# agordon/fastx_toolkit

Hardware: AMD Instinct MI355X
Metric: Mreads/s (150 bp) quality-trim+filter (higher is better)
Workload: dtype u8

## Files before the change

fastx_toolkit_amd/build.py:

```python
import os
import shutil
import subprocess
import sys

PKG = os.path.dirname(os.path.abspath(__file__))
ROOT = os.path.dirname(PKG)
CSRC = os.path.join(PKG, "csrc")
HOST = os.path.join(PKG, "host")
LIBFXG = os.path.join(PKG, "libfxg.so")

HIPCC_FLAGS = ["--offload-arch=gfx950", "-O3", "-std=c++17", "-ffp-contract=off", "-fPIC", "-shared"]


def _newer(target, deps):
    if not os.path.exists(target):
        return True
    t = os.path.getmtime(target)
    return any(os.path.getmtime(d) > t for d in deps if os.path.exists(d))


def hipcc():
    exe = shutil.which("hipcc") or "/opt/rocm/bin/hipcc"
    if not os.path.exists(exe):
        raise RuntimeError("hipcc not found: the gfx950 engine cannot be built")
    return exe


def check_exec_zero(so):
    tool = os.path.join(ROOT, "scripts", "check_exec_zero.py")
    p = subprocess.run([sys.executable, tool, so], stdout=subprocess.PIPE, stderr=subprocess.STDOUT, text=True)
    if p.returncode not in (0, 1):
        raise RuntimeError("%s NOT CHECKED: scripts/check_exec_zero.py could not read the library's ISA (exit code %d); that is a broken check, "
                           "not a finding, and a library that was not checked is not accepted.\n%s" % (so, p.returncode, p.stdout[-3000:]))
    if p.returncode != 0:
        raise RuntimeError("%s REJECTED: vector/memory code runs with EXEC = 0 at the exit of a lane-divergent loop (compiler bug, DESIGN.md section 3).\n"
                           "Change the register budget of the named instance (fxg_clip_waves / __launch_bounds__) or its source and rebuild.\n%s" % (so, p.stdout[-3000:]))


CLIP_UNITS = 7


def compile_engine(out, extra_flags=(), check=True):
    tmp = out + ".new"
    objdir = os.path.join(ROOT, "build", "engine_" + os.path.basename(out).replace(".", "_"))
    os.makedirs(objdir, exist_ok=True)
    cflags = [f for f in HIPCC_FLAGS if f != "-shared"] + list(extra_flags) + ["-c"]
    units = [("fxg_engine.hip", ["-DFXG_SPLIT"], os.path.join(objdir, "engine.o"))]
    units += [("fxg_engine_clip.hip", ["-DFXG_CLIP_TU=%d" % k], os.path.join(objdir, "clip%d.o" % k)) for k in range(1, CLIP_UNITS + 1)]
    procs = [(src, subprocess.Popen([hipcc()] + cflags + defs + [os.path.join(CSRC, src), "-o", obj])) for src, defs, obj in units]
    failed = [src for src, p in procs if p.wait() != 0]
    if failed:
        raise RuntimeError("hipcc failed on %s" % ", ".join(failed))
    subprocess.check_call([hipcc(), "--offload-arch=gfx950", "-fPIC", "-shared"] + [obj for _, _, obj in units] + ["-o", tmp])
    if check:
        try:
            check_exec_zero(tmp)
        except Exception:
            os.replace(tmp, out + ".rejected")
            raise
    os.replace(tmp, out)
    return out


def build_engine(force=False):
    deps = [os.path.join(CSRC, f) for f in os.listdir(CSRC)] + [os.path.join(ROOT, "include", "fxg.h")]
    if force or _newer(LIBFXG, deps):
        compile_engine(LIBFXG)
    return LIBFXG


def build_host(force=False):
    mk = os.path.join(HOST, "Makefile")
    if os.path.exists(mk):
        subprocess.check_call(["make", "-s", "-C", HOST] + (["-B"] if force else []))


def build_all(force=False):
    build_engine(force)
    build_host(force)
    return LIBFXG
```

fastx_toolkit_amd/csrc/fxg_device.h:

```cpp
#pragma once
#include <hip/hip_runtime.h>
#include <stdint.h>
#include <cstdio>
#include <cstring>

#include "../../include/fxg.h"

typedef unsigned int       u32;
typedef unsigned long long u64;
typedef unsigned int u32x4 __attribute__((ext_vector_type(4)));

#define FXG_HD __host__ __device__ __forceinline__
#define FXG_PLAN_FAIL(...) do { snprintf(err, cap, __VA_ARGS__); return FXG_E_INVALID; } while (0)
static inline int fxg_text_check_len(unsigned long long text_len, char *err, size_t cap) { if (text_len > 0xFFFFFFF0ull) FXG_PLAN_FAIL("text block too large (%llu bytes)", text_len); return FXG_OK; }
static inline bool fxg_text_lpr_ok(int lpr) { return lpr == 4 || lpr == 2; }

#if defined(FXG_ABLATION) || defined(FXG_DBG_BITS)
#define FXG_DBG(a, bit) ((a).debug & (bit))
#else
#define FXG_DBG(a, bit) 0u
#endif

#define FXG_BLOCK 256
#define FXG_WAVES (FXG_BLOCK / 64)
// ... 410 lines not shown
    return lane < 2u ? fxg_granule_load(a.pfx + 2 * (u64)tile + lane) : ((u64)a.tag << FXG_TAG_SHIFT);
}
__device__ __forceinline__ void fxg_wait_prefix(const FxgKArgs &a, u32 tile, u64 peek, u64 *bc)
{
    const u32 lane = fxg_lane();
    u64 v = peek;
    u32 spins = 0;
    const u64 t0 = __builtin_amdgcn_s_memrealtime();
    while (__ballot((u32)(v >> FXG_TAG_SHIFT) != a.tag) != 0ull) {
        __builtin_amdgcn_s_sleep(1);
        if (lane < 2u) v = fxg_granule_load(a.pfx + 2 * (u64)tile + lane);
        if ((++spins & 255u) == 0u && fxg_spin_expired(a, t0)) break;
    }
    const bool ok = __ballot((u32)(v >> FXG_TAG_SHIFT) != a.tag) == 0ull;
    if (lane < 2u) bc[lane] = ok ? FXG_TAG_VALUE(v) : ~0ull;
}

#ifndef FXG_POLL_SLEEP
#define FXG_POLL_SLEEP 1
#endif
__device__ __forceinline__ void fxg_wait_prefix_wave(const FxgKArgs &a, u32 tile, u64 *bc)
{
    const u32 lane = fxg_lane();
    u64 v = fxg_peek_prefix(a, tile);
    u32 spins = 0;
    const u64 t0 = __builtin_amdgcn_s_memrealtime();
    while (__ballot((u32)(v >> FXG_TAG_SHIFT) != a.tag) != 0ull) {
        __builtin_amdgcn_s_sleep(FXG_POLL_SLEEP);
        if (lane < 2u) v = fxg_granule_load(a.pfx + 2 * (u64)tile + lane);
        if ((++spins & 255u) == 0u && fxg_spin_expired(a, t0)) break;
    }
    const bool ok = __ballot((u32)(v >> FXG_TAG_SHIFT) != a.tag) == 0ull;
    v = ok ? FXG_TAG_VALUE(v) : ~0ull;
    bc[0] = ((u64)(u32)__builtin_amdgcn_readlane((int)(v >> 32), 0) << 32) | (u32)__builtin_amdgcn_readlane((int)(u32)v, 0);
    bc[1] = ((u64)(u32)__builtin_amdgcn_readlane((int)(v >> 32), 1) << 32) | (u32)__builtin_amdgcn_readlane((int)(u32)v, 1);
}

template <int TW = FXG_TWAVES>
__device__ __forceinline__ void fxg_block_scan2(u32 c, u32 b, u32 *scratch, u32 *ex_c, u32 *ex_b, u32 *tot_c, u32 *tot_b)
{
    const u32 lane = fxg_lane(), wave = threadIdx.x >> 6;
    const u32 ic = fxg_wave_scan_dpp(c), ib = fxg_wave_scan_dpp(b);
    if constexpr (TW == 1) {
        *ex_c = ic - c; *ex_b = ib - b;
        *tot_c = (u32)__builtin_amdgcn_readlane((int)ic, 63); *tot_b = (u32)__builtin_amdgcn_readlane((int)ib, 63);
        return;
    }
    if (lane == 63) { scratch[wave] = ic; scratch[TW + wave] = ib; }
    __syncthreads();
    u32 oc = 0, ob = 0, sc = 0, sb = 0;
#pragma unroll
    for (int w = 0; w < TW; ++w) {
// ... 181 lines not shown
```

fastx_toolkit_amd/csrc/fxg_engine.hip:

```cpp
#include "fxg_host.h"
#include "fxg_text.h"
#include "fxg_history.h"
#include "fxg_stats.h"
#include "fxg_fallback.h"
#include "fxg_barcode.h"
#include "fxg_reflow.h"

extern "C" int fxg_abi_version(void) { return FXG_ABI_VERSION; }

extern "C" int fxg_ctx_create(int device_id, fxg_ctx **out)
{
    if (!out) return FXG_E_INVALID;
    *out = nullptr;
    int ndev = 0;
    if (hipGetDeviceCount(&ndev) != hipSuccess || ndev <= 0 || device_id < 0 || device_id >= ndev) return FXG_E_HIP;
    fxg_ctx *c = (fxg_ctx *)calloc(1, sizeof(fxg_ctx));
    if (!c) return FXG_E_NOMEM;
    c->device = device_id;
    hipDeviceProp_t prop;
    if (hipSetDevice(device_id) != hipSuccess || hipGetDeviceProperties(&prop, device_id) != hipSuccess ||
        hipStreamCreateWithFlags(&c->own_stream, hipStreamNonBlocking) != hipSuccess) { fxg_ctx_destroy(c); return FXG_E_HIP; }
    c->cus = prop.multiProcessorCount;
    c->stream = c->own_stream;
    { const char *e = getenv("FXG_BLOCKS_PER_CU"); c->env_blocks_per_cu = (e && atoi(e) > 0 && atoi(e) <= 16) ? atoi(e) : 0; }
// ... 162 lines not shown
    }
    if (hist) {
        FXG_HIP(c, hipSetDevice(c->device));
        FXG_TRY(fxg_hist_prepass(c, in, estride, pl));
    }
    c->fb_req.valid = 0;
    if (pl.ka.compact) { c->fb_req.in = *in; c->fb_req.p = *p; c->fb_req.out = *out; c->fb_req.hist = hist; c->fb_req.estride = estride; c->fb_req.valid = 1; }
    return fxg_launch_plan(c, pl, (u64 *)out->counters);
}

static int fxg_launch_clip(fxg_ctx *c, FxgPlan &pl, u64 *ctr)
{
    int rc;
#define FXG_CLIP_TRY_UNIT(K) if ((rc = FXG_CLIP_UNIT_FN(K)(c, pl, ctr)) != FXG_CLIP_NOT_MINE) return rc;
    FXG_CLIP_FOR_UNITS(FXG_CLIP_TRY_UNIT)
#undef FXG_CLIP_TRY_UNIT
    return fxg_fail(c, FXG_E_INVALID, "no clip instance %d", pl.amax);
}

static int fxg_launch_plan(fxg_ctx *c, FxgPlan &pl, u64 *ctr)
{
    if (pl.rows_nw) {
        if (pl.rows_h == 2) {
            if (pl.rows_nw == 26) return fxg_launch_tiles(c, fxg_kernel_rows<26, 2>, "fxg_kernel_rows<26,2> qtrim+qfilter", pl.ka, pl.lds, ctr, 64u, true);
            return fxg_launch_tiles(c, fxg_kernel_rows<38, 2>, "fxg_kernel_rows<38,2> qtrim+qfilter", pl.ka, pl.lds, ctr, 64u, true);
        }
        switch (pl.rows_nw) {
        case 10: return fxg_launch_tiles(c, fxg_kernel_rows_multi<10, 4>, "fxg_kernel_rows_multi<10,4> qtrim+qfilter", pl.ka, pl.lds, ctr, 64u, true);
        case 14: return fxg_launch_tiles(c, fxg_kernel_rows_multi<14, 3>, "fxg_kernel_rows_multi<14,3> qtrim+qfilter", pl.ka, pl.lds, ctr, 64u, true);
        case 20: return fxg_launch_tiles(c, fxg_kernel_rows_multi<20, 2>, "fxg_kernel_rows_multi<20,2> qtrim+qfilter", pl.ka, pl.lds, ctr, 64u, true);
        case 26: return fxg_launch_tiles(c, fxg_kernel_rows<26>, "fxg_kernel_rows<26> qtrim+qfilter", pl.ka, pl.lds, ctr, 64u, true);
        default: return fxg_launch_tiles(c, fxg_kernel_rows<38>, "fxg_kernel_rows<38> qtrim+qfilter", pl.ka, pl.lds, ctr, 64u, true);
        }
    }
    if (pl.group_a) {
        if (pl.amax == 0) return fxg_launch_tiles(c, fxg_kernel_tiles<0, 0>, "fxg_kernel_tiles<0,0> qtrim+qfilter", pl.ka, pl.lds, ctr);
        return fxg_launch_clip(c, pl, ctr);
    }
    if (pl.mask) return fxg_launch_tiles(c, fxg_kernel_tiles<0, 3>, "fxg_kernel_tiles<0,3> mask", pl.ka, pl.lds, ctr);
    if (pl.artifacts) return fxg_launch_tiles(c, fxg_kernel_tiles<0, 4>, "fxg_kernel_tiles<0,4> base census", pl.ka, pl.lds, ctr);
    if (pl.rev && pl.ka.rev_dw) return fxg_launch_tiles(c, fxg_kernel_tiles<0, 5>, "fxg_kernel_tiles<0,5> revcomp[+ftrim], dword-aligned windows", pl.ka, pl.lds, ctr);
    if (pl.rev) return fxg_launch_tiles(c, fxg_kernel_tiles<0, 2>, "fxg_kernel_tiles<0,2> revcomp[+ftrim]", pl.ka, pl.lds, ctr);
    return fxg_launch_tiles(c, fxg_kernel_tiles<0, 1>, "fxg_kernel_tiles<0,1> ftrim", pl.ka, pl.lds, ctr);
}

extern "C" int fxg_run_quality_stats(fxg_ctx *c, const fxg_batch *in, uint64_t *d_hist, uint32_t hist_cols)
{
    if (!c) return FXG_E_INVALID;
    FXG_TRY(fxg_stats_check(in, d_hist, hist_cols, c->err, sizeof c->err));
    if (in->n == 0) return FXG_OK;
    FXG_HIP(c, hipSetDevice(c->device));
    u64 nwg = (in->n + 255) / 256;
    if (nwg > (u64)c->cus) nwg = (u64)c->cus;
    FxgStatsArgs a = fxg_stats_args(in, d_hist, hist_cols, (u32)nwg);
    const size_t need = (size_t)a.nwg * FXG_QS_PART_WORDS;
// ... 523 lines not shown
```

fastx_toolkit_amd/csrc/fxg_engine_clip.hip:

```cpp
#include "fxg_host.h"

#define FXG_CLIP_LAUNCH(K, NAME) return fxg_launch_tiles(c, K, NAME, pl.ka, pl.lds, ctr, pl.block, false, pl.ck_per_wg);
#define FXG_CLIP_CASE_PACKED(N) case -N: FXG_CLIP_LAUNCH((pl.ka.clip_global ? fxg_kernel_tiles<-N, 0, true> : fxg_kernel_tiles<-N, 0, false>), "fxg_kernel_tiles<-" #N ",0> clip(packed)[+qtrim+qfilter]")
#define FXG_CLIP_CASE_GENERAL(N) case N: FXG_CLIP_LAUNCH((fxg_kernel_tiles<N, 0>), "fxg_kernel_tiles<" #N ",0> clip[+qtrim+qfilter]")
#define FXG_CLIP_DEFINE_UNIT(K) \
    int FXG_CLIP_UNIT_FN(K)(fxg_ctx *c, FxgPlan &pl, u64 *ctr) { switch (pl.amax) { FXG_CLIP_UNIT(K)(FXG_CLIP_CASE_PACKED, FXG_CLIP_CASE_GENERAL) default: return FXG_CLIP_NOT_MINE; } }

#ifdef FXG_CLIP_TU
FXG_CLIP_DEFINE_UNIT(FXG_CLIP_TU)
#else
FXG_CLIP_FOR_UNITS(FXG_CLIP_DEFINE_UNIT)
#endif
```

fastx_toolkit_amd/csrc/fxg_host.h:

```cpp
#pragma once
#include <hip/hip_runtime.h>

#include <dlfcn.h>
#include <fcntl.h>
#include <cerrno>
#include <cstdarg>
#include <cstdio>
#include <cstdlib>
#include <cstring>
#include <unistd.h>

#include "fxg_plan.h"
#include "fxg_rows.h"

struct FxgTextState;

struct fxg_ctx {
    int device;
    int cus;
    hipStream_t own_stream;
    hipStream_t stream;
    hipEvent_t ev0, ev1;
#define FXG_KEV_RING 64
    hipEvent_t kev0[FXG_KEV_RING], kev1[FXG_KEV_RING];
// ... 89 lines not shown
template <typename K>
static int fxg_kernel_fit(fxg_ctx *c, K kernel, const char *kname, u32 lds, int *per_cu, u32 block = FXG_TBLOCK)
{
    for (int i = 0; i < 8; ++i)
        if (c->attr_kernel[i] == (void *)kernel && c->attr_lds[i] == lds) { *per_cu = c->attr_per_cu[i]; return FXG_OK; }
    int k = -1;
    for (int i = 0; i < 32; ++i) { if (c->lds_kernel[i] == (void *)kernel) { k = i; break; } if (!c->lds_kernel[i] && k < 0) k = i; }
    if (k < 0 || c->lds_kernel[k] != (void *)kernel || c->lds_max[k] < lds) {
        FXG_HIP(c, hipFuncSetAttribute((const void *)kernel, hipFuncAttributeMaxDynamicSharedMemorySize, (int)lds));
        if (k >= 0) { c->lds_kernel[k] = (void *)kernel; c->lds_max[k] = lds; }
    }
    FXG_HIP(c, hipOccupancyMaxActiveBlocksPerMultiprocessor(per_cu, kernel, (int)block, lds));
    if (*per_cu < 1) return fxg_fail(c, FXG_E_INVALID, "%s does not fit on a CU (lds=%u)", kname, lds);
    int slot = -1;
    for (int i = 0; i < 8; ++i) if (!c->attr_kernel[i]) { slot = i; break; }
    if (slot < 0) { slot = c->attr_next; c->attr_next = (c->attr_next + 1) % 8; }
    c->attr_kernel[slot] = (void *)kernel; c->attr_lds[slot] = lds; c->attr_per_cu[slot] = *per_cu;
    return FXG_OK;
}

#define FXG_STATUS_WORDS(cap) (3 * (size_t)(cap) + 2 * ((size_t)(cap) / 256 + 2))

template <typename K>
static int fxg_launch_tiles(fxg_ctx *c, K kernel, const char *kname, FxgKArgs &ka, u32 lds, u64 *counters, u32 block = FXG_TBLOCK, bool rows_kernel = false, u64 ck_per_wg = 0)
{
    FXG_HIP(c, hipSetDevice(c->device));
    int per_cu = 0;
    FXG_TRY(fxg_kernel_fit(c, kernel, kname, lds, &per_cu, block));
    const int most = block == 64u ? 16 : 8;
    int use = per_cu > most ? most : per_cu;
    if (c->env_blocks_per_cu > 0) use = c->env_blocks_per_cu;
    u64 workers = (u64)c->cus * (u64)use;
    if (c->env_workers > 0 && workers > (u64)c->env_workers) workers = (u64)c->env_workers;
    if (workers > ka.ntiles) workers = ka.ntiles;
    if (workers < 1) workers = 1;
    ka.nscan = !ka.compact ? 0u : (rows_kernel && workers >= 64u * FXG_ROWS_NSCAN ? (u32)FXG_ROWS_NSCAN : 1u);
    if (ka.compact && rows_kernel && c->env_nscan > 0) ka.nscan = (u32)c->env_nscan;
    const u64 grid = workers + ka.nscan;

    if (ka.compact) {
        bool fresh = false;
        const size_t cap = (size_t)ka.ntiles + (size_t)ka.ntiles / 4 + 1024;
        FXG_TRY(fxg_ws_grow(c, c->status, c->status_cap, ka.ntiles, cap, &fresh, FXG_STATUS_WORDS(cap) * sizeof(u64)));
        c->epoch = c->epoch >= 255u ? 1u : c->epoch + 1u;
        if (fresh || c->epoch == 1u) FXG_HIP(c, hipMemsetAsync(c->status, 0, FXG_STATUS_WORDS(c->status_cap) * sizeof(u64), c->stream));
        ka.agg = c->status;
        ka.pfx = c->status + c->status_cap;
        ka.bbase = c->status + 3 * c->status_cap;
        ka.tag = c->epoch;
    }
    ka.clip_ck = nullptr;
    if (ck_per_wg) {
// ... 32 lines not shown
```

fastx_toolkit_amd/csrc/fxg_plan.h:

```cpp
#pragma once
#include <cstdio>
#include <cstdlib>
#include <cstring>

#include "fxg_clip_instances.h"
#include "fxg_kernels.h"
#include "fxg_rows.h"

static_assert(fxg_clip_bucket(1) != 0 && fxg_clip_bucket(FXG_MAX_ADAPTER) != 0, "every adapter length the plan accepts needs a packed clip instance");

struct FxgPlan {
    FxgKArgs ka;
    bool group_a;
    bool clip, use_q, rev;
    bool mask, artifacts;
    int  amax;
    u32  lds;
    int  rows_nw;
    int  rows_h;
    int  rows_r;
    u32  block;
    u64  ck_per_wg;
};

static inline int fxg_clampi(long long v, int lo, int hi) { return v < lo ? lo : (v > hi ? hi : (int)v); }

static inline u32 fxg_pick_tile(u32 stride, bool clip, u32 block = FXG_TBLOCK)
{
    const u64 budget = clip ? 60ull * 1024 : 20ull * 1024;
    u32 T = block;
    const char *env = getenv("FXG_TILE");
    if (env && atoi(env) >= 1 && atoi(env) <= (int)block && (atoi(env) & (atoi(env) - 1)) == 0) return (u32)atoi(env);
    while (T > 1 && (u64)T * stride > budget) T >>= 1;
    return T;
}

static inline FxgLds fxg_plan_layout(const FxgPlan *pl)
{
    const FxgKArgs &ka = pl->ka;
    return pl->group_a ? fxg_lds_layout(ka.tile_reads, ka.stride, fxg_bitmap_count(ka, pl->use_q, pl->clip), (pl->clip && !ka.clip_global) ? ka.clip_stride : 0u, pl->clip ? ka.depth : 2u, pl->clip,
                                        (pl->clip && fxg_clip_uses_ptab(pl->amax)) ? fxg_ptab_bytes(ka.clip_ptab_rows, ka.clip_ptab_stride) : 0u)
         : pl->mask ? fxg_lds_layout(ka.tile_reads, ka.stride, 2u, 0u)
         : pl->artifacts ? fxg_lds_layout(ka.tile_reads, ka.stride, 4u, 0u) : fxg_lds_layout(ka.tile_reads, ka.stride, 0u, 0u);
// ... 66 lines not shown
        pl->amax = -b;
        if (two_pass_k) pl->ck_per_wg = (u64)FXG_CK_SLOTS * (u64)b * FXG_TBLOCK;
        ka.clip_ptab_cols = kform ? ((u32)b + 3u) & ~3u : 16u;
        ka.clip_ptab_stride = fxg_ptab_stride(ka.clip_ptab_cols);
        ka.clip_ptab_dia1 = kform ? FXG_K_DIA1 : FXG_PK_DIA1;
        if (kform && ka.clip_ptab_rows > FXG_PTAB_MAX_ROWS_K) {
            pl->amax = ka.alen <= 32 ? 32 : ka.alen <= 64 ? 64 : 100;
            pl->ck_per_wg = 0;
        }
    }
    pl->rows_nw = 0; pl->rows_h = 1; pl->rows_r = 1;
    {
        const int want = getenv("FXG_ROWS") ? atoi(getenv("FXG_ROWS")) : 1;
        const u32 top = want >= 2 ? 304u : 208u;
        if (ga && !pl->clip && ka.compact && in->stride >= 80u && in->stride <= top && want != 0) {
            pl->rows_h = in->stride <= 152u ? 1 : 2;
            pl->rows_nw = in->stride <= 104u * (u32)pl->rows_h ? 26 : 38;
        } else if (ga && !pl->clip && ka.compact && in->stride >= 28u && in->stride < 80u && want != 0) {
            if (in->stride <= 40u) { pl->rows_nw = 10; pl->rows_r = 4; }
            else if (in->stride <= 56u) { pl->rows_nw = 14; pl->rows_r = 3; }
            else { pl->rows_nw = 20; pl->rows_r = 2; }
        }
    }
    pl->block = pl->rows_nw ? 64u : (ga && pl->amax < 0 && pl->amax >= -16) ? (u32)FXG_CLIP_TBLOCK : (u32)FXG_TBLOCK;
    ka.clip_global = 0u;
    u32 T = pl->rows_nw ? 64u * (u32)pl->rows_r / (u32)pl->rows_h : fxg_pick_tile(pl->clip ? ka.clip_stride : in->stride, pl->clip, pl->block);
    if (pl->clip && pl->amax < 0 && (pl->amax >= -16 || pl->ck_per_wg != 0) && clip_stride == 0u && (ka.clip_stride & 3u) == 0u && ((uintptr_t)ka.clip_src & 3u) == 0u) {
        ka.tile_reads = T; ka.depth = 2u;
        const bool cramped = T < pl->block || (156u * 1024u) / fxg_plan_lds(pl) < 3u;
        const char *e = getenv("FXG_CLIP_GLOBAL");
        ka.clip_global = (e ? atoi(e) != 0 : cramped) ? 1u : 0u;
        if (ka.clip_global) T = pl->block;
    }
    const u64 ntiles = (in->n + T - 1) / T;
    if (ntiles > 0x7FFFFFFFull || in->n > 0xFFFFFFFFull) FXG_PLAN_FAIL("batch too large (%llu reads): split it", (unsigned long long)in->n);
    ka.tile_reads = T; ka.ntiles = (u32)ntiles;
    ka.rev_dw = 0u;
    if ((st & FXG_STAGE_REVCOMP) && !in->len && (T & 3u) == 0u) {
        u32 start = 0, cur = in->fixed_len;
        if (st & FXG_STAGE_FTRIM) {
            if (p->ft_last != 0 && (u32)p->ft_last < cur) cur = (u32)p->ft_last;
            if (p->ft_first != 1 && cur >= (u32)p->ft_first) { start = (u32)p->ft_first - 1u; cur -= start; }
        }
        if ((st & FXG_STAGE_FTRIM_END) && cur > p->ft_trim_end) cur -= p->ft_trim_end;
        const u32 A = (in->stride + cur) & 3u, C = (in->fixed_len - start) & 3u;
        ka.rev_dw = ((A == 0u && C != 0u) || (A == 2u && (C & 1u))) ? 1u : 0u;
// ... 36 lines not shown
```

fastx_toolkit_amd/csrc/fxg_rows.h:

```cpp
#pragma once
#include "fxg_kernels.h"

#define FXG_ROWS_T 64u
#ifndef FXG_ROWS_LB
#define FXG_ROWS_LB 3
#endif
#ifndef FXG_ROWS_SCAN_K
#define FXG_ROWS_SCAN_K 8
#endif
#ifndef FXG_ROWS_LD_AUX
#define FXG_ROWS_LD_AUX 2
#endif
#ifndef FXG_ROWS_NSCAN
#define FXG_ROWS_NSCAN 8
#endif
#ifndef FXG_ROWS_SPARSE_BASES
#define FXG_ROWS_SPARSE_BASES 1
#endif
#define FXG_ROWS_SPARSE_MULTI (FXG_ROWS_SPARSE_BASES >= 2)

__host__ __device__ inline u32 fxg_rows_lds(u32 stride, u32 lanes_per_read = 1u, u32 reads_per_lane = 1u) { return fxg_r16(FXG_ROWS_T * reads_per_lane / lanes_per_read * stride) + 176u; }

template <int NW>
FXG_HD void fxg_rows_bits(const u32 (&row)[NW], u32 K, u32 (&M)[(NW * 4 + 31) / 32])
{
#pragma unroll
    for (int p = 0; p < (NW + 1) / 2; ++p) {
        const u32 f0 = fxg_ge_flags(row[2 * p], K), f1 = 2 * p + 1 < NW ? fxg_ge_flags(row[2 * p + 1], K) : 0u;
#ifndef FXG_HOST_EMULATION
// ... 225 lines not shown
    const u32 first = sh ? 1u : 0u, end = (sh + totb) >> 4;
    const u32 s2 = (16u - sh) & 15u, qd = s2 >> 2, r = s2 & 3u;
    const int a8 = (int)(((base - sh) >> 4) & 7u);
    for (int ii = (int)lane - a8; ii < (int)end; ii += 64) {
        if (ii < (int)first) continue;
        const u32 i = (u32)ii;
        const u32x4 *src = reinterpret_cast<const u32x4 *>(obuf + ((i - first) << 4));
        const u32x4 v0 = src[0], v1 = src[1];
        u32 w0, w1, w2, w3, w4;
        if (qd == 0u)      { w0 = v0.x; w1 = v0.y; w2 = v0.z; w3 = v0.w; w4 = v1.x; }
        else if (qd == 1u) { w0 = v0.y; w1 = v0.z; w2 = v0.w; w3 = v1.x; w4 = v1.y; }
        else if (qd == 2u) { w0 = v0.z; w1 = v0.w; w2 = v1.x; w3 = v1.y; w4 = v1.z; }
        else               { w0 = v0.w; w1 = v1.x; w2 = v1.y; w3 = v1.z; w4 = v1.w; }
        const u32x4 o = {__builtin_amdgcn_alignbyte(w1, w0, r), __builtin_amdgcn_alignbyte(w2, w1, r), __builtin_amdgcn_alignbyte(w3, w2, r), __builtin_amdgcn_alignbyte(w4, w3, r)};
        fxg_st16_stream(g0 + ((u64)i << 4), o);
    }
    const bool whole = end > first;
    const u32 hb = whole ? (sh ? 16u - sh : 0u) : totb;
    const u32 ts = whole ? (end << 4) - sh : totb;
    if (lane < hb) out[base + lane] = obuf[lane];
    if (ts + lane < totb) out[base + ts + lane] = obuf[ts + lane];
}

#ifdef FXG_ABLATION
#define FXG_PHASE(i) do { const u64 now_ = __builtin_amdgcn_s_memrealtime(); ph[i] += now_ - pt; pt = now_; } while (0)
#else
#define FXG_PHASE(i) do { } while (0)
#endif

template <int NW, int H = 1>
__global__ __launch_bounds__(64, FXG_ROWS_LB) void fxg_kernel_rows(const FxgKArgs a)
{
    constexpr u32 TR = FXG_ROWS_T / (u32)H, HB = 4u * (u32)NW;
    extern __shared__ __attribute__((aligned(16))) unsigned char smem[];
    fxg_lds_u8 *lsm = (fxg_lds_u8 *)smem;
    u32 lane = threadIdx.x;
    const u32 stride = a.stride;
#if FXG_ROWS_SPARSE_BASES
    const u32 magic = fxg_rows_magic(stride);
#endif
    u32 role = 0;
    if (lane == 0) role = atomicAdd(a.role, 1u);
    role = (u32)__builtin_amdgcn_readfirstlane((int)role);
    if (role < a.nscan) { if (a.nscan == 1u) fxg_scanner_k<FXG_ROWS_SCAN_K>(a); else fxg_scanner_multi<FXG_ROWS_SCAN_K>(a, role); return; }
    const u32 G = a.ticket_groups, grp = blockIdx.x % G;
    u32 *my_ticket = a.ticket + grp * FXG_TICKET_STRIDE;
    u32 tk = 0;
    if (lane == 0) tk = atomicAdd(my_ticket, 1u);
    u32 cur = (u32)__builtin_amdgcn_readfirstlane((int)tk) * G + grp;
    u64 t_in = 0, t_kept = 0, t_bases = 0, t_qtrim = 0, t_qfilter = 0;
#ifdef FXG_ABLATION
    u64 ph[8] = {0, 0, 0, 0, 0, 0, 0, 0}, pt = __builtin_amdgcn_s_memrealtime();
#endif
    u32 qp[NW];
    u32 p_info = 0, p_exc = 0, p_totb = 0, pend = FXG_NO_TILE;
    for (;;) {
        asm volatile("" : "+v"(lane));
        const bool havec = cur < a.ntiles, havep = pend != FXG_NO_TILE;
        u32 q[NW];
        u32 c_info = 0, c_exc = 0, c_totb = 0;
        if (havec) {
            const u32 r0 = cur * TR;
            const u64 left = a.n - (u64)r0;
            const u32 nreads = left < (u64)TR ? (u32)left : TR;
            const u64 tb = (u64)r0 * stride;
            const u32 tbytes = nreads * stride;
            const u32 rd = lane / (u32)H, hf = lane % (u32)H;
            fxg_rows_fetch<NW>(a.qual, tb, tbytes, lsm, lane);
            fxg_rows_landed();
            FXG_PHASE(0);
            fxg_rows_read<NW>(smem, rd * stride + hf * HB, q);
            FXG_WAVE_SYNC();
            u32 keep = 0, olen = 0, word = 0;
            if constexpr (H == 1) {
                if (lane < nreads) word = fxg_rows_decide<NW>(a, q, r0 + lane, &keep, &olen);
            } else {
                constexpr int NM = (NW * 4 + 31) / 32;
                const bool live = rd < nreads;
                const u32 rl = live ? (a.len ? (u32)a.len[r0 + rd] : a.fixed_len) : 0u;
                u32 G[NM];
                const u32 kp = fxg_rows_piece_last<NW>(a, q, fxg_rows_piece_len(rl, HB, hf), G);
                const u32 ko = (u32)__builtin_amdgcn_mov_dpp((int)kp, 0xB1, 0xf, 0xf, true);
                const u32 k_lo = hf ? ko : kp, k_hi = hf ? kp : ko;
                const u32 k = k_hi ? HB + k_hi : k_lo;
                const u32 cl = (a.stages & FXG_STAGE_QTRIM) ? k : rl;
                const u32 lp = fxg_rows_piece_low<NW>(a, q, G, fxg_rows_piece_len(cl, HB, hf));
                const u32 lo_ = (u32)__builtin_amdgcn_mov_dpp((int)lp, 0xB1, 0xf, 0xf, true);
                u32 rlen = 0;
                word = fxg_rows_verdict(a, rl, k, lp + lo_, &keep, &rlen);
                if (!live) { keep = 0; word = 0; }
                if (live && hf == 0u) a.res[r0 + rd] = word;
                olen = keep ? fxg_rows_piece_len(rlen, HB, hf) : 0u;
                if (hf) word = 0;
            }
            {
                const u32 why = (H == 1 ? lane < nreads : rd < nreads) ? (word >> 17) & 0xFu : 0u;
                t_qtrim += (u64)__builtin_popcountll(__ballot(why == FXG_R_QTRIM));
                t_qfilter += (u64)__builtin_popcountll(__ballot(why == FXG_R_QFILTER));
            }
            const u32 mine = keep ? ((hf == 0u ? 1u << 16 : 0u) | olen) : 0u;
            const u32 inc = fxg_wave_scan_dpp(mine);
            const u32 tot = (u32)__builtin_amdgcn_readlane((int)inc, 63);
            const u32 totc = tot >> 16;
            c_totb = tot & 0xFFFFu;
            c_exc = (inc - mine) >> 16;
            c_info = ((keep && (H == 1 || hf == 0u || olen)) ? 1u << 31 : 0u) | (olen << 16) | ((inc - mine) & 0xFFFFu);
            if (lane == 0) fxg_publish_total(a, cur, totc, c_totb);
            t_in += nreads; t_kept += totc; t_bases += c_totb;
            FXG_PHASE(1);
        }
        u64 bc[2] = {0, 0};
        if (havep) {
            if (!FXG_DBG(a, 2u)) fxg_wait_prefix_wave(a, pend, bc); else { bc[0] = (u64)pend * TR; bc[1] = bc[0] * stride; }
            FXG_PHASE(2);
        }
        u32 nxt = 0;
        if (havec && lane == 0) nxt = atomicAdd(my_ticket, 1u);
        if (havep) {
            const u32 r0 = pend * TR;
            const u64 left = a.n - (u64)r0;
            const u32 nreads = left < (u64)TR ? (u32)left : TR;
            const u64 tb = (u64)r0 * stride;
            const u32 tbytes = nreads * stride;
            const u32 rd = lane / (u32)H, hf = lane % (u32)H;
            const bool placed = bc[0] != ~0ull;
            const u32 keep = placed ? p_info >> 31 : 0u, olen = (p_info >> 16) & 0x7FFFu, exb = p_info & 0xFFFFu;
            const bool fast = __ballot(keep && olen < 4u) == 0ull;
            if (keep && !FXG_DBG(a, 64u)) fxg_rows_pack<NW>(smem, exb, qp, olen, fast);
            FXG_WAVE_SYNC();
            FXG_PHASE(6);
            if (placed && !FXG_DBG(a, 1u)) fxg_rows_flush(a.out_qual, bc[1], p_totb, smem, lane);
// ... 17 lines not shown
#endif
                fxg_rows_fetch<NW, FXG_ROWS_SPARSE_BASES != 0>(a.bases, tb, tbytes, lsm, lane, need);
                fxg_rows_landed();
                FXG_PHASE(4);
                fxg_rows_read<NW>(smem, rd * stride + hf * HB, b);
                FXG_WAVE_SYNC();
                if (keep && !FXG_DBG(a, 64u)) fxg_rows_pack<NW>(smem, exb, b, olen, fast);
                FXG_WAVE_SYNC();
                FXG_PHASE(7);
                if (placed && !FXG_DBG(a, 1u)) fxg_rows_flush(a.out_bases, bc[1], p_totb, smem, lane);
                FXG_WAVE_SYNC();
            }
            FXG_PHASE(5);
        }
        if (!havec) break;
#pragma unroll
        for (int k = 0; k < NW; ++k) qp[k] = q[k];
        p_info = c_info; p_exc = c_exc; p_totb = c_totb; pend = cur;
        cur = (u32)__builtin_amdgcn_readfirstlane((int)nxt) * G + grp;
    }
#ifdef FXG_ABLATION
    if (lane == 0) for (int i = 0; i < 8; ++i) atomicAdd(reinterpret_cast<u64 *>(a.errflag + 10) + i, ph[i]);
#endif
    if (lane == 0) {
        if (t_in) atomicAdd(&a.tally[0], t_in);
        if (t_kept) atomicAdd(&a.tally[1], t_kept);
        if (t_bases) atomicAdd(&a.tally[2], t_bases);
        if (t_qtrim) atomicAdd(&a.tally[4 + FXG_R_QTRIM], t_qtrim);
        if (t_qfilter) atomicAdd(&a.tally[4 + FXG_R_QFILTER], t_qfilter);
    }
}
template <int NW, int R>
__global__ __launch_bounds__(64, FXG_ROWS_LB) void fxg_kernel_rows_multi(const FxgKArgs a)
{
    constexpr u32 TR = FXG_ROWS_T * (u32)R;
    extern __shared__ __attribute__((aligned(16))) unsigned char smem[];
    fxg_lds_u8 *lsm = (fxg_lds_u8 *)smem;
    u32 lane = threadIdx.x;
    const u32 stride = a.stride;
#if FXG_ROWS_SPARSE_MULTI
    const u32 magic = fxg_rows_magic(stride);
#endif
    u32 role = 0;
    if (lane == 0) role = atomicAdd(a.role, 1u);
    role = (u32)__builtin_amdgcn_readfirstlane((int)role);
    if (role < a.nscan) { if (a.nscan == 1u) fxg_scanner_k<FXG_ROWS_SCAN_K>(a); else fxg_scanner_multi<FXG_ROWS_SCAN_K>(a, role); return; }
    const u32 G = a.ticket_groups, grp = blockIdx.x % G;
    u32 *my_ticket = a.ticket + grp * FXG_TICKET_STRIDE;
    u32 tk = 0;
    if (lane == 0) tk = atomicAdd(my_ticket, 1u);
    u32 cur = (u32)__builtin_amdgcn_readfirstlane((int)tk) * G + grp;
    u64 t_in = 0, t_kept = 0, t_bases = 0, t_qtrim = 0, t_qfilter = 0;
    u32 qp[R][NW];
    u32 p_info[R], p_exc[R], p_totb = 0, pend = FXG_NO_TILE;
#pragma unroll
    for (int j = 0; j < R; ++j) { p_info[j] = 0u; p_exc[j] = 0u; }
    for (;;) {
        asm volatile("" : "+v"(lane));
        const bool havec = cur < a.ntiles, havep = pend != FXG_NO_TILE;
        u32 q[R][NW];
        u32 c_info[R], c_exc[R], c_totb = 0;
#pragma unroll
        for (int j = 0; j < R; ++j) { c_info[j] = 0u; c_exc[j] = 0u; }
        if (havec) {
            const u32 r0 = cur * TR;
            const u64 left = a.n - (u64)r0;
            const u32 nreads = left < (u64)TR ? (u32)left : TR;
            const u64 tb = (u64)r0 * stride;
            const u32 tbytes = nreads * stride;
            fxg_rows_fetch<NW * R>(a.qual, tb, tbytes, lsm, lane);
            fxg_rows_landed();
#pragma unroll
            for (int j = 0; j < R; ++j) fxg_rows_read<NW>(smem, ((u32)j * FXG_ROWS_T + lane) * stride, q[j]);
            FXG_WAVE_SYNC();
            u32 base = 0;
#pragma unroll
            for (int j = 0; j < R; ++j) {
                const u32 rd = (u32)j * FXG_ROWS_T + lane;
                u32 keep = 0, olen = 0, word = 0;
                if (rd < nreads) word = fxg_rows_decide<NW>(a, q[j], r0 + rd, &keep, &olen);
                const u32 why = rd < nreads ? (word >> 17) & 0xFu : 0u;
                t_qtrim += (u64)__builtin_popcountll(__ballot(why == FXG_R_QTRIM));
                t_qfilter += (u64)__builtin_popcountll(__ballot(why == FXG_R_QFILTER));
                const u32 mine = keep ? ((1u << 16) | olen) : 0u;
                const u32 inc = fxg_wave_scan_dpp(mine);
                const u32 ex = inc - mine + base;
                base += (u32)__builtin_amdgcn_readlane((int)inc, 63);
                c_exc[j] = ex >> 16;
                c_info[j] = (keep ? 1u << 31 : 0u) | (olen << 16) | (ex & 0xFFFFu);
            }
            const u32 totc = base >> 16;
            c_totb = base & 0xFFFFu;
            if (lane == 0) fxg_publish_total(a, cur, totc, c_totb);
            t_in += nreads; t_kept += totc; t_bases += c_totb;
        }
        u64 bc[2] = {0, 0};
        if (havep) fxg_wait_prefix_wave(a, pend, bc);
        u32 nxt = 0;
        if (havec && lane == 0) nxt = atomicAdd(my_ticket, 1u);
        if (havep) {
            const u32 r0 = pend * TR;
            const u64 left = a.n - (u64)r0;
            const u32 nreads = left < (u64)TR ? (u32)left : TR;
            const u64 tb = (u64)r0 * stride;
            const u32 tbytes = nreads * stride;
            const bool placed = bc[0] != ~0ull;
            u64 shortm = 0;
#pragma unroll
            for (int j = 0; j < R; ++j) shortm |= __ballot(placed && (p_info[j] >> 31) && ((p_info[j] >> 16) & 0x7FFFu) < 4u);
            const bool fast = shortm == 0ull;
#pragma unroll
            for (int j = 0; j < R; ++j) {
                const u32 keep = placed ? p_info[j] >> 31 : 0u, olen = (p_info[j] >> 16) & 0x7FFFu, exb = p_info[j] & 0xFFFFu;
                if (keep) fxg_rows_pack<NW>(smem, exb, qp[j], olen, fast);
            }
            FXG_WAVE_SYNC();
            if (placed) fxg_rows_flush(a.out_qual, bc[1], p_totb, smem, lane);
// ... 17 lines not shown
#pragma unroll
                for (int j = 0; j < R; ++j) fxg_rows_read<NW>(smem, ((u32)j * FXG_ROWS_T + lane) * stride, b[j]);
                FXG_WAVE_SYNC();
#pragma unroll
                for (int j = 0; j < R; ++j) {
                    const u32 keep = placed ? p_info[j] >> 31 : 0u, olen = (p_info[j] >> 16) & 0x7FFFu, exb = p_info[j] & 0xFFFFu;
                    if (keep) fxg_rows_pack<NW>(smem, exb, b[j], olen, fast);
                }
                FXG_WAVE_SYNC();
                if (placed) fxg_rows_flush(a.out_bases, bc[1], p_totb, smem, lane);
                FXG_WAVE_SYNC();
            }
        }
        if (!havec) break;
#pragma unroll
        for (int j = 0; j < R; ++j) {
#pragma unroll
            for (int k = 0; k < NW; ++k) qp[j][k] = q[j][k];
            p_info[j] = c_info[j]; p_exc[j] = c_exc[j];
        }
        p_totb = c_totb; pend = cur;
        cur = (u32)__builtin_amdgcn_readfirstlane((int)nxt) * G + grp;
    }
    if (lane == 0) {
        if (t_in) atomicAdd(&a.tally[0], t_in);
        if (t_kept) atomicAdd(&a.tally[1], t_kept);
        if (t_bases) atomicAdd(&a.tally[2], t_bases);
        if (t_qtrim) atomicAdd(&a.tally[4 + FXG_R_QTRIM], t_qtrim);
        if (t_qfilter) atomicAdd(&a.tally[4 + FXG_R_QFILTER], t_qfilter);
    }
}
#endif
```

Baseline: 13070.

## Tune per-instance rows-kernel occupancy, scalarize prefix polling, and slim tally counters

Gives each rows-kernel instance its own launch-bounds wave count and blocks-per-CU cap through a table, replacing the fixed 16-per-CU cap for the rows path. The prefix wait now builds a uniform global pointer with readfirstlane and polls with relaxed agent-scope atomic loads. Per-wave tallies become u32 counters: the qfilter count is derived as in minus kept minus qtrim, dropping one ballot per row, and tile totals are read as scalars. The build also records compiler resource-usage remarks to a JSON file. The per-CU caps (12 or 16) and the derived qfilter count could change occupancy or tally results if the cap is worse or the counts don't add up.

Result: no change. 13060 (median of 2 runs) (-0.0%).

```diff
diff --git a/fastx_toolkit_amd/build.py b/fastx_toolkit_amd/build.py
--- a/fastx_toolkit_amd/build.py
+++ b/fastx_toolkit_amd/build.py
@@ -1,4 +1,6 @@
+import json
 import os
+import re
 import shutil
 import subprocess
 import sys
@@ -8,6 +10,7 @@
 CSRC = os.path.join(PKG, "csrc")
 HOST = os.path.join(PKG, "host")
 LIBFXG = os.path.join(PKG, "libfxg.so")
+RESOURCES = os.path.join(PKG, "libfxg.resources.json")
 
 HIPCC_FLAGS = ["--offload-arch=gfx950", "-O3", "-std=c++17", "-ffp-contract=off", "-fPIC", "-shared"]
 
@@ -37,6 +40,40 @@
                            "Change the register budget of the named instance (fxg_clip_waves / __launch_bounds__) or its source and rebuild.\n%s" % (so, p.stdout[-3000:]))
 
 
+RESOURCE_REMARKS = "-Rpass-analysis=kernel-resource-usage"
+_REMARK = re.compile(r"remark:\s+([A-Za-z ]+?)(?: \[[^\]]*\])?: (\S+) \[-Rpass-analysis=kernel-resource-usage\]")
+_FIELDS = {"VGPRs": "vgprs", "AGPRs": "agprs", "TotalSGPRs": "sgprs", "ScratchSize": "scratch_bytes", "Occupancy": "occupancy",
+           "VGPRs Spill": "vgpr_spills", "SGPRs Spill": "sgpr_spills"}
+
+
+def _demangle(symbols):
+    tool = next((t for t in (os.path.join(os.path.dirname(os.path.realpath(hipcc())), "..", "llvm", "bin", "llvm-cxxfilt"),
+                             shutil.which("llvm-cxxfilt"), shutil.which("c++filt")) if t and os.path.exists(t)), None)
+    if not tool or not symbols:
+        return list(symbols)
+    p = subprocess.run([tool] + list(symbols), stdout=subprocess.PIPE, text=True)
+    names = p.stdout.split("\n")[:len(symbols)]
+    return names if p.returncode == 0 and len(names) == len(symbols) else list(symbols)
+
+
+def kernel_resources(logs):
+    found = {}
+    for unit, log in logs:
+        cur = None
+        with open(log, errors="replace") as f:
+            for line in f:
+                m = _REMARK.search(line)
+                if not m:
+                    continue
+                key, val = m.groups()
+                if key == "Function Name":
+                    cur = found.setdefault(val, {"symbol": val, "unit": unit})
+                elif cur is not None and key in _FIELDS:
+                    cur[_FIELDS[key]] = int(val)
+    symbols = sorted(found)
+    return {name: found[sym] for sym, name in zip(symbols, _demangle(symbols))}
+
+
 CLIP_UNITS = 7
 
 
@@ -44,13 +81,16 @@
     tmp = out + ".new"
     objdir = os.path.join(ROOT, "build", "engine_" + os.path.basename(out).replace(".", "_"))
     os.makedirs(objdir, exist_ok=True)
-    cflags = [f for f in HIPCC_FLAGS if f != "-shared"] + list(extra_flags) + ["-c"]
+    cflags = [f for f in HIPCC_FLAGS if f != "-shared"] + list(extra_flags) + [RESOURCE_REMARKS, "-c"]
     units = [("fxg_engine.hip", ["-DFXG_SPLIT"], os.path.join(objdir, "engine.o"))]
     units += [("fxg_engine_clip.hip", ["-DFXG_CLIP_TU=%d" % k], os.path.join(objdir, "clip%d.o" % k)) for k in range(1, CLIP_UNITS + 1)]
-    procs = [(src, subprocess.Popen([hipcc()] + cflags + defs + [os.path.join(CSRC, src), "-o", obj])) for src, defs, obj in units]
-    failed = [src for src, p in procs if p.wait() != 0]
+    procs = [(src, obj, subprocess.Popen([hipcc()] + cflags + defs + [os.path.join(CSRC, src), "-o", obj], stderr=open(obj + ".log", "w"))) for src, defs, obj in units]
+    failed = [(src, obj) for src, obj, p in procs if p.wait() != 0]
     if failed:
-        raise RuntimeError("hipcc failed on %s" % ", ".join(failed))
+        for _, obj in failed:
+            with open(obj + ".log", errors="replace") as f:
+                sys.stderr.write("".join(line for line in f if RESOURCE_REMARKS not in line)[-6000:])
+        raise RuntimeError("hipcc failed on %s" % ", ".join(src for src, _ in failed))
     subprocess.check_call([hipcc(), "--offload-arch=gfx950", "-fPIC", "-shared"] + [obj for _, _, obj in units] + ["-o", tmp])
     if check:
         try:
@@ -59,12 +99,22 @@
             os.replace(tmp, out + ".rejected")
             raise
     os.replace(tmp, out)
+    res = kernel_resources([(os.path.basename(obj)[:-2], obj + ".log") for _, _, obj in units])
+    if not res:
+        raise RuntimeError("%s: the compiler reported no kernel's resource usage (%s)" % (out, RESOURCE_REMARKS))
+    with open(resources_path(out) + ".new", "w") as f:
+        json.dump({"flags": cflags, "kernels": res}, f, indent=1, sort_keys=True)
+    os.replace(resources_path(out) + ".new", resources_path(out))
     return out
+
+
+def resources_path(so):
+    return so[:-len(".so")] + ".resources.json" if so.endswith(".so") else so + ".resources.json"
 
 
 def build_engine(force=False):
     deps = [os.path.join(CSRC, f) for f in os.listdir(CSRC)] + [os.path.join(ROOT, "include", "fxg.h")]
-    if force or _newer(LIBFXG, deps):
+    if force or _newer(LIBFXG, deps) or not os.path.exists(RESOURCES):
         compile_engine(LIBFXG)
     return LIBFXG
 
diff --git a/fastx_toolkit_amd/csrc/fxg_device.h b/fastx_toolkit_amd/csrc/fxg_device.h
--- a/fastx_toolkit_amd/csrc/fxg_device.h
+++ b/fastx_toolkit_amd/csrc/fxg_device.h
@@ -456,12 +456,16 @@
 __device__ __forceinline__ void fxg_wait_prefix_wave(const FxgKArgs &a, u32 tile, u64 *bc)
 {
     const u32 lane = fxg_lane();
-    u64 v = fxg_peek_prefix(a, tile);
+    typedef __attribute__((address_space(1))) u64 global_u64;
+    const u64 at = (u64)(uintptr_t)(a.pfx + 2 * (u64)tile);
+    global_u64 *g = (global_u64 *)(uintptr_t)(((u64)(u32)__builtin_amdgcn_readfirstlane((int)(u32)(at >> 32)) << 32) | (u32)__builtin_amdgcn_readfirstlane((int)(u32)at));
+    const auto granule = [g, lane]() { return (u64)__hip_atomic_load(g + lane, __ATOMIC_RELAXED, __HIP_MEMORY_SCOPE_AGENT); };
+    u64 v = lane < 2u ? granule() : ((u64)a.tag << FXG_TAG_SHIFT);
     u32 spins = 0;
     const u64 t0 = __builtin_amdgcn_s_memrealtime();
     while (__ballot((u32)(v >> FXG_TAG_SHIFT) != a.tag) != 0ull) {
         __builtin_amdgcn_s_sleep(FXG_POLL_SLEEP);
-        if (lane < 2u) v = fxg_granule_load(a.pfx + 2 * (u64)tile + lane);
+        if (lane < 2u) v = granule();
         if ((++spins & 255u) == 0u && fxg_spin_expired(a, t0)) break;
     }
     const bool ok = __ballot((u32)(v >> FXG_TAG_SHIFT) != a.tag) == 0ull;
diff --git a/fastx_toolkit_amd/csrc/fxg_engine.hip b/fastx_toolkit_amd/csrc/fxg_engine.hip
--- a/fastx_toolkit_amd/csrc/fxg_engine.hip
+++ b/fastx_toolkit_amd/csrc/fxg_engine.hip
@@ -208,15 +208,15 @@
 {
     if (pl.rows_nw) {
         if (pl.rows_h == 2) {
-            if (pl.rows_nw == 26) return fxg_launch_tiles(c, fxg_kernel_rows<26, 2>, "fxg_kernel_rows<26,2> qtrim+qfilter", pl.ka, pl.lds, ctr, 64u, true);
-            return fxg_launch_tiles(c, fxg_kernel_rows<38, 2>, "fxg_kernel_rows<38,2> qtrim+qfilter", pl.ka, pl.lds, ctr, 64u, true);
+            if (pl.rows_nw == 26) return fxg_launch_tiles(c, fxg_kernel_rows<26, 2>, "fxg_kernel_rows<26,2> qtrim+qfilter", pl.ka, pl.lds, ctr, 64u, pl.rows_per_cu);
+            return fxg_launch_tiles(c, fxg_kernel_rows<38, 2>, "fxg_kernel_rows<38,2> qtrim+qfilter", pl.ka, pl.lds, ctr, 64u, pl.rows_per_cu);
         }
         switch (pl.rows_nw) {
-        case 10: return fxg_launch_tiles(c, fxg_kernel_rows_multi<10, 4>, "fxg_kernel_rows_multi<10,4> qtrim+qfilter", pl.ka, pl.lds, ctr, 64u, true);
-        case 14: return fxg_launch_tiles(c, fxg_kernel_rows_multi<14, 3>, "fxg_kernel_rows_multi<14,3> qtrim+qfilter", pl.ka, pl.lds, ctr, 64u, true);
-        case 20: return fxg_launch_tiles(c, fxg_kernel_rows_multi<20, 2>, "fxg_kernel_rows_multi<20,2> qtrim+qfilter", pl.ka, pl.lds, ctr, 64u, true);
-        case 26: return fxg_launch_tiles(c, fxg_kernel_rows<26>, "fxg_kernel_rows<26> qtrim+qfilter", pl.ka, pl.lds, ctr, 64u, true);
-        default: return fxg_launch_tiles(c, fxg_kernel_rows<38>, "fxg_kernel_rows<38> qtrim+qfilter", pl.ka, pl.lds, ctr, 64u, true);
+        case 10: return fxg_launch_tiles(c, fxg_kernel_rows_multi<10, 4>, "fxg_kernel_rows_multi<10,4> qtrim+qfilter", pl.ka, pl.lds, ctr, 64u, pl.rows_per_cu);
+        case 14: return fxg_launch_tiles(c, fxg_kernel_rows_multi<14, 3>, "fxg_kernel_rows_multi<14,3> qtrim+qfilter", pl.ka, pl.lds, ctr, 64u, pl.rows_per_cu);
+        case 20: return fxg_launch_tiles(c, fxg_kernel_rows_multi<20, 2>, "fxg_kernel_rows_multi<20,2> qtrim+qfilter", pl.ka, pl.lds, ctr, 64u, pl.rows_per_cu);
+        case 26: return fxg_launch_tiles(c, fxg_kernel_rows<26>, "fxg_kernel_rows<26> qtrim+qfilter", pl.ka, pl.lds, ctr, 64u, pl.rows_per_cu);
+        default: return fxg_launch_tiles(c, fxg_kernel_rows<38>, "fxg_kernel_rows<38> qtrim+qfilter", pl.ka, pl.lds, ctr, 64u, pl.rows_per_cu);
         }
     }
     if (pl.group_a) {
diff --git a/fastx_toolkit_amd/csrc/fxg_engine_clip.hip b/fastx_toolkit_amd/csrc/fxg_engine_clip.hip
--- a/fastx_toolkit_amd/csrc/fxg_engine_clip.hip
+++ b/fastx_toolkit_amd/csrc/fxg_engine_clip.hip
@@ -1,6 +1,6 @@
 #include "fxg_host.h"
 
-#define FXG_CLIP_LAUNCH(K, NAME) return fxg_launch_tiles(c, K, NAME, pl.ka, pl.lds, ctr, pl.block, false, pl.ck_per_wg);
+#define FXG_CLIP_LAUNCH(K, NAME) return fxg_launch_tiles(c, K, NAME, pl.ka, pl.lds, ctr, pl.block, 0, pl.ck_per_wg);
 #define FXG_CLIP_CASE_PACKED(N) case -N: FXG_CLIP_LAUNCH((pl.ka.clip_global ? fxg_kernel_tiles<-N, 0, true> : fxg_kernel_tiles<-N, 0, false>), "fxg_kernel_tiles<-" #N ",0> clip(packed)[+qtrim+qfilter]")
 #define FXG_CLIP_CASE_GENERAL(N) case N: FXG_CLIP_LAUNCH((fxg_kernel_tiles<N, 0>), "fxg_kernel_tiles<" #N ",0> clip[+qtrim+qfilter]")
 #define FXG_CLIP_DEFINE_UNIT(K) \
diff --git a/fastx_toolkit_amd/csrc/fxg_host.h b/fastx_toolkit_amd/csrc/fxg_host.h
--- a/fastx_toolkit_amd/csrc/fxg_host.h
+++ b/fastx_toolkit_amd/csrc/fxg_host.h
@@ -135,12 +135,13 @@
 #define FXG_STATUS_WORDS(cap) (3 * (size_t)(cap) + 2 * ((size_t)(cap) / 256 + 2))
 
 template <typename K>
-static int fxg_launch_tiles(fxg_ctx *c, K kernel, const char *kname, FxgKArgs &ka, u32 lds, u64 *counters, u32 block = FXG_TBLOCK, bool rows_kernel = false, u64 ck_per_wg = 0)
+static int fxg_launch_tiles(fxg_ctx *c, K kernel, const char *kname, FxgKArgs &ka, u32 lds, u64 *counters, u32 block = FXG_TBLOCK, int rows_per_cu = 0, u64 ck_per_wg = 0)
 {
     FXG_HIP(c, hipSetDevice(c->device));
     int per_cu = 0;
     FXG_TRY(fxg_kernel_fit(c, kernel, kname, lds, &per_cu, block));
-    const int most = block == 64u ? 16 : 8;
+    const bool rows_kernel = rows_per_cu != 0;
+    const int most = rows_kernel ? rows_per_cu : block == 64u ? 16 : 8;
     int use = per_cu > most ? most : per_cu;
     if (c->env_blocks_per_cu > 0) use = c->env_blocks_per_cu;
     u64 workers = (u64)c->cus * (u64)use;
diff --git a/fastx_toolkit_amd/csrc/fxg_plan.h b/fastx_toolkit_amd/csrc/fxg_plan.h
--- a/fastx_toolkit_amd/csrc/fxg_plan.h
+++ b/fastx_toolkit_amd/csrc/fxg_plan.h
@@ -19,6 +19,7 @@
     int  rows_nw;
     int  rows_h;
     int  rows_r;
+    int  rows_per_cu;
     u32  block;
     u64  ck_per_wg;
 };
@@ -131,6 +132,7 @@
             else { pl->rows_nw = 20; pl->rows_r = 2; }
         }
     }
+    pl->rows_per_cu = !pl->rows_nw ? 0 : pl->rows_r > 1 ? fxg_rows_per_cu(true, pl->rows_nw, pl->rows_r) : fxg_rows_per_cu(false, pl->rows_nw, pl->rows_h);
     pl->block = pl->rows_nw ? 64u : (ga && pl->amax < 0 && pl->amax >= -16) ? (u32)FXG_CLIP_TBLOCK : (u32)FXG_TBLOCK;
     ka.clip_global = 0u;
     u32 T = pl->rows_nw ? 64u * (u32)pl->rows_r / (u32)pl->rows_h : fxg_pick_tile(pl->clip ? ka.clip_stride : in->stride, pl->clip, pl->block);
diff --git a/fastx_toolkit_amd/csrc/fxg_rows.h b/fastx_toolkit_amd/csrc/fxg_rows.h
--- a/fastx_toolkit_amd/csrc/fxg_rows.h
+++ b/fastx_toolkit_amd/csrc/fxg_rows.h
@@ -2,9 +2,30 @@
 #include "fxg_kernels.h"
 
 #define FXG_ROWS_T 64u
-#ifndef FXG_ROWS_LB
-#define FXG_ROWS_LB 3
-#endif
+#define FXG_ROWS_INSTANCES(X) \
+    X(0, 38, 1, 3, 12) \
+    X(0, 38, 2, 3, 12) \
+    X(0, 26, 1, 3, 16) \
+    X(0, 26, 2, 3, 16) \
+    X(1, 10, 4, 3, 12) \
+    X(1, 14, 3, 3, 12) \
+    X(1, 20, 2, 3, 12)
+#define FXG_ROWS_PICK_LB(M, NW, X_, LB, WG) if (multi == (M != 0) && nw == NW && x == X_) return LB;
+#define FXG_ROWS_PICK_WG(M, NW, X_, LB, WG) if (multi == (M != 0) && nw == NW && x == X_) return WG;
+constexpr int fxg_rows_waves(bool multi, int nw, int x)
+{
+#ifdef FXG_ROWS_LB
+    return FXG_ROWS_LB;
+#else
+    FXG_ROWS_INSTANCES(FXG_ROWS_PICK_LB)
+    return 3;
+#endif
+}
+constexpr int fxg_rows_per_cu(bool multi, int nw, int x)
+{
+    FXG_ROWS_INSTANCES(FXG_ROWS_PICK_WG)
+    return 16;
+}
 #ifndef FXG_ROWS_SCAN_K
 #define FXG_ROWS_SCAN_K 8
 #endif
@@ -276,6 +297,26 @@
     if (ts + lane < totb) out[base + ts + lane] = obuf[ts + lane];
 }
 
+struct FxgRowsTally {
+    u32 in = 0, kept = 0, qtrim = 0;
+    u64 bytes = 0;
+    __device__ __forceinline__ void dropped_by_trim(bool mine) { qtrim += (u32)__builtin_popcountll(__ballot(mine)); }
+    __device__ __forceinline__ void tile(u32 nreads, u32 tot)
+    {
+        const u32 t = (u32)__builtin_amdgcn_readfirstlane((int)tot), nr = (u32)__builtin_amdgcn_readfirstlane((int)nreads);
+        in += nr; kept += t >> 16; bytes += t & 0xFFFFu;
+    }
+    __device__ __forceinline__ void add_to(const FxgKArgs &a) const
+    {
+        const u32 qfilter = in - kept - qtrim;
+        if (in) atomicAdd(&a.tally[0], (u64)in);
+        if (kept) atomicAdd(&a.tally[1], (u64)kept);
+        if (bytes) atomicAdd(&a.tally[2], bytes);
+        if (qtrim) atomicAdd(&a.tally[4 + FXG_R_QTRIM], (u64)qtrim);
+        if (qfilter) atomicAdd(&a.tally[4 + FXG_R_QFILTER], (u64)qfilter);
+    }
+};
+
 #ifdef FXG_ABLATION
 #define FXG_PHASE(i) do { const u64 now_ = __builtin_amdgcn_s_memrealtime(); ph[i] += now_ - pt; pt = now_; } while (0)
 #else
@@ -283,7 +324,7 @@
 #endif
 
 template <int NW, int H = 1>
-__global__ __launch_bounds__(64, FXG_ROWS_LB) void fxg_kernel_rows(const FxgKArgs a)
+__global__ __launch_bounds__(64, fxg_rows_waves(false, NW, H)) void fxg_kernel_rows(const FxgKArgs a)
 {
     constexpr u32 TR = FXG_ROWS_T / (u32)H, HB = 4u * (u32)NW;
     extern __shared__ __attribute__((aligned(16))) unsigned char smem[];
@@ -302,7 +343,7 @@
     u32 tk = 0;
     if (lane == 0) tk = atomicAdd(my_ticket, 1u);
     u32 cur = (u32)__builtin_amdgcn_readfirstlane((int)tk) * G + grp;
-    u64 t_in = 0, t_kept = 0, t_bases = 0, t_qtrim = 0, t_qfilter = 0;
+    FxgRowsTally tl;
 #ifdef FXG_ABLATION
     u64 ph[8] = {0, 0, 0, 0, 0, 0, 0, 0}, pt = __builtin_amdgcn_s_memrealtime();
 #endif
@@ -347,11 +388,7 @@
                 olen = keep ? fxg_rows_piece_len(rlen, HB, hf) : 0u;
                 if (hf) word = 0;
             }
-            {
-                const u32 why = (H == 1 ? lane < nreads : rd < nreads) ? (word >> 17) & 0xFu : 0u;
-                t_qtrim += (u64)__builtin_popcountll(__ballot(why == FXG_R_QTRIM));
-                t_qfilter += (u64)__builtin_popcountll(__ballot(why == FXG_R_QFILTER));
-            }
+            tl.dropped_by_trim((H == 1 ? lane < nreads : rd < nreads) && ((word >> 17) & 0xFu) == FXG_R_QTRIM);
             const u32 mine = keep ? ((hf == 0u ? 1u << 16 : 0u) | olen) : 0u;
             const u32 inc = fxg_wave_scan_dpp(mine);
             const u32 tot = (u32)__builtin_amdgcn_readlane((int)inc, 63);
@@ -360,7 +397,7 @@
             c_exc = (inc - mine) >> 16;
             c_info = ((keep && (H == 1 || hf == 0u || olen)) ? 1u << 31 : 0u) | (olen << 16) | ((inc - mine) & 0xFFFFu);
             if (lane == 0) fxg_publish_total(a, cur, totc, c_totb);
-            t_in += nreads; t_kept += totc; t_bases += c_totb;
+            tl.tile(nreads, tot);
             FXG_PHASE(1);
         }
         u64 bc[2] = {0, 0};
@@ -424,16 +461,10 @@
 #ifdef FXG_ABLATION
     if (lane == 0) for (int i = 0; i < 8; ++i) atomicAdd(reinterpret_cast<u64 *>(a.errflag + 10) + i, ph[i]);
 #endif
-    if (lane == 0) {
-        if (t_in) atomicAdd(&a.tally[0], t_in);
-        if (t_kept) atomicAdd(&a.tally[1], t_kept);
-        if (t_bases) atomicAdd(&a.tally[2], t_bases);
-        if (t_qtrim) atomicAdd(&a.tally[4 + FXG_R_QTRIM], t_qtrim);
-        if (t_qfilter) atomicAdd(&a.tally[4 + FXG_R_QFILTER], t_qfilter);
-    }
+    if (lane == 0) tl.add_to(a);
 }
 template <int NW, int R>
-__global__ __launch_bounds__(64, FXG_ROWS_LB) void fxg_kernel_rows_multi(const FxgKArgs a)
+__global__ __launch_bounds__(64, fxg_rows_waves(true, NW, R)) void fxg_kernel_rows_multi(const FxgKArgs a)
 {
     constexpr u32 TR = FXG_ROWS_T * (u32)R;
     extern __shared__ __attribute__((aligned(16))) unsigned char smem[];
@@ -452,7 +483,7 @@
     u32 tk = 0;
     if (lane == 0) tk = atomicAdd(my_ticket, 1u);
     u32 cur = (u32)__builtin_amdgcn_readfirstlane((int)tk) * G + grp;
-    u64 t_in = 0, t_kept = 0, t_bases = 0, t_qtrim = 0, t_qfilter = 0;
+    FxgRowsTally tl;
     u32 qp[R][NW];
     u32 p_info[R], p_exc[R], p_totb = 0, pend = FXG_NO_TILE;
 #pragma unroll
@@ -481,9 +512,7 @@
                 const u32 rd = (u32)j * FXG_ROWS_T + lane;
                 u32 keep = 0, olen = 0, word = 0;
                 if (rd < nreads) word = fxg_rows_decide<NW>(a, q[j], r0 + rd, &keep, &olen);
-                const u32 why = rd < nreads ? (word >> 17) & 0xFu : 0u;
-                t_qtrim += (u64)__builtin_popcountll(__ballot(why == FXG_R_QTRIM));
-                t_qfilter += (u64)__builtin_popcountll(__ballot(why == FXG_R_QFILTER));
+                tl.dropped_by_trim(rd < nreads && ((word >> 17) & 0xFu) == FXG_R_QTRIM);
                 const u32 mine = keep ? ((1u << 16) | olen) : 0u;
                 const u32 inc = fxg_wave_scan_dpp(mine);
                 const u32 ex = inc - mine + base;
@@ -494,7 +523,7 @@
             const u32 totc = base >> 16;
             c_totb = base & 0xFFFFu;
             if (lane == 0) fxg_publish_total(a, cur, totc, c_totb);
-            t_in += nreads; t_kept += totc; t_bases += c_totb;
+            tl.tile(nreads, base);
         }
         u64 bc[2] = {0, 0};
         if (havep) fxg_wait_prefix_wave(a, pend, bc);
@@ -558,12 +587,6 @@
         p_totb = c_totb; pend = cur;
         cur = (u32)__builtin_amdgcn_readfirstlane((int)nxt) * G + grp;
     }
-    if (lane == 0) {
-        if (t_in) atomicAdd(&a.tally[0], t_in);
-        if (t_kept) atomicAdd(&a.tally[1], t_kept);
-        if (t_bases) atomicAdd(&a.tally[2], t_bases);
-        if (t_qtrim) atomicAdd(&a.tally[4 + FXG_R_QTRIM], t_qtrim);
-        if (t_qfilter) atomicAdd(&a.tally[4 + FXG_R_QFILTER], t_qfilter);
-    }
-}
-#endif
+    if (lane == 0) tl.add_to(a);
+}
+#endif
```
